# astra-vision/rain-rendering

Hardware: AMD Instinct MI355X
Metric: rainy frames/sec @ 1242x375, 100 mm/hr (higher is better)
Workload: dtype f64 alpha/mask, f32 colour

## Files before the change

rain-rendering_amd/csrc/rainhip.hip:

```cpp
#include <hip/hip_runtime.h>

#include <dlfcn.h>

#include <cstddef>
#include <cstdio>
#include <cstdlib>
#include <algorithm>
#include <cstring>
#include <string>
#include <mutex>
#include <unordered_map>
#include <vector>

#include "rainhip.h"
#include "rr_device.h"
#include "rr_prepass.h"
#include "rr_deflate.h"
#include "rr_pngrows.h"
#include "rr_particles.h"

using namespace rr;

namespace {

// ... 88 lines not shown
    out[1] = __hiloint2double((int)q.d, (int)q.c);
    out[2] = __hiloint2double((int)q.f, (int)q.e);
  } else if (kind == 1) {
    out[0] = (double)__uint_as_float(q.a);
    out[1] = (double)__uint_as_float(q.b);
    out[2] = (double)__uint_as_float(q.c);
  } else {
    out[0] = (double)q.a / 255.0;
    out[1] = (double)q.b / 255.0;
    out[2] = (double)q.c / 255.0;
  }
}
__device__ inline int bg_kind(const FrameDesc& fr) { return (fr.in_types & RR_IN_BG_U8) ? 2 : ((fr.in_types & RR_IN_BG_F32) ? 1 : 0); }
__device__ inline int rainy_kind(const FrameDesc& fr) {
  if (fr.rainy_bg == fr.bg) return bg_kind(fr);
  return (fr.in_types & RR_IN_RAINY_U8) ? 2 : ((fr.in_types & RR_IN_RAINY_F32) ? 1 : 0);
}
typedef float float2_u __attribute__((ext_vector_type(2), aligned(4)));
typedef float float4_u __attribute__((ext_vector_type(4), aligned(4)));

__device__ inline void wave_lds_sync() {
  __builtin_amdgcn_fence(__ATOMIC_ACQ_REL, "wavefront");
  __builtin_amdgcn_wave_barrier();
}

#ifdef RR_PHASES
__device__ unsigned long long g_phase[8][8];
#define PH_DECL unsigned long long ph_t0_ = __builtin_readcyclecounter(), ph_acc_[8] = {0, 0, 0, 0, 0, 0, 0, 0};
#define PH_WAITVM asm volatile("s_waitcnt vmcnt(0)" ::: "memory");
#define PH(k)                                                   \
  {                                                             \
    const unsigned long long ph_n_ = __builtin_readcyclecounter(); \
    ph_acc_[k] += ph_n_ - ph_t0_;                               \
    ph_t0_ = ph_n_;                                             \
  }
#define PH_FLUSH(kid)                                           \
  if ((threadIdx.x & 63) == 0) {                                \
    for (int ph_q_ = 0; ph_q_ < 8; ph_q_++)                     \
      if (ph_acc_[ph_q_]) atomicAdd(&g_phase[kid][ph_q_], ph_acc_[ph_q_]); \
  }
#define PH_PARAMS , unsigned long long& ph_t0_, unsigned long long (&ph_acc_)[8]
#define PH_PASS , ph_t0_, ph_acc_
#define PH_COUNT(k) ph_acc_[k] += 1;
#else
#define PH_PARAMS
#define PH_PASS
#define PH_COUNT(k)
#define PH_DECL
#define PH_WAITVM
#define PH(k)
#define PH_FLUSH(kid)
#endif

struct Scratch {
  DropPlan* plan;
  CompRec* comp;
  CompRec32* comp32;
  int32_t* poly;
  int32_t* npts;
  int64_t* sizes;
  double* prefix;
  double* fband;
  double* arena;
  double* partial;
  double* means;
  int64_t* arena_need;
  int32_t* overflow;
  unsigned long long* need_max;
  int32_t* list_rot;
  int32_t* rot_total;
  int32_t* list_gen;
  int32_t* list_slow;
  int4* blur_items;
  int32_t* list_small;
  double* colpart;
  double* wtab;
  double* wtab_big;
  const uint8_t* tex_pad;
  const int64_t* tex_poff;
  uint4* fov_erec;
  uint32_t* fov_pix;
  int32_t* fov_list;
  int32_t* fov_list_n;
  uint4* fov_rec;
  int32_t* fov_order;
  int32_t* fov_slot;
  int32_t fov_slots;
  uint8_t* blended;
  int32_t* pad_first;
  int32_t* eff_first;
  uint32_t* spans;
  int4* bbox;
  uint16_t* clist;
  int32_t* ccount;
  int32_t* counts;
  int32_t* list_big;
  int32_t* big_off;
  int32_t* bigs_list;
  int32_t* bigs_n;
  uint4* tkey;
  uint4* lrec;
  int32_t* canon;
  int32_t* htab;
  int32_t blur_bx, blur_by;
  int32_t* rows_list;
  int32_t* rows_n;
  int32_t* rows_hist;
  unsigned long long* rows_cost;
  int32_t* rows_next;
  int32_t* rows_bounds;
  int32_t* rows_fbase;
  int32_t* rows_sorted;
  const uint8_t* tex_pair;
  const int64_t* tex_qoff;
  int32_t colpart_f32;
  int32_t rows_on, n_tex;
  int32_t big_on, n_buckets;
};

__global__ __launch_bounds__(256) void k_env_prefix(const FrameDesc* frames, Dims dm, double* prefix) {
  const int lane = threadIdx.x & 63;
  const int row = blockIdx.x * 4 + (threadIdx.x >> 6), f = blockIdx.y;
  if (row >= dm.He) return;
  const FrameDesc& fr = frames[f];
  const int We = dm.We;
  const bool e32 = (fr.in_types & RR_IN_ENV_F32) != 0;
  const global_ptr<const double> env = as_global(static_cast<const double*>(fr.env)) + (int64_t)row * We * 3;
  const global_ptr<const double> om = as_global(static_cast<const double*>(fr.omega)) + (int64_t)row * We;
// ... 885 lines not shown
    int32_t* dst = pass == 0 ? slot : order;
    const int shift = 16 + 8 * pass;
    for (int e = t; e < 256 * FOV_SORT_WAVES; e += 64 * FOV_SORT_WAVES) s_cnt[e] = 0u;
    __syncthreads();
    for (int p = p0 + lane; p < p1; p += 64) {
      const int idx = pass == 0 ? p : src[p];
      atomicAdd(&s_cnt[((recs[idx].w >> shift) & 255u) * FOV_SORT_WAVES + wave], 1u);
    }
    __syncthreads();
    {
      uint32_t c[4], sum = 0u;
#pragma unroll
      for (int k = 0; k < 4; k++) { c[k] = s_cnt[4 * t + k]; sum += c[k]; }
      const uint32_t incl = wave_incl_scan_u32(sum);
      if (lane == 63) s_wtot[wave] = incl;
      __syncthreads();
      uint32_t run = incl - sum;
      for (int w = 0; w < wave; w++) run += s_wtot[w];
#pragma unroll
      for (int k = 0; k < 4; k++) { s_cnt[4 * t + k] = run; run += c[k]; }
    }
    __syncthreads();
    for (int c = p0; c < p1; c += 64) {
      const int p = c + lane;
      const bool valid = p < p1;
      const int idx = valid ? (pass == 0 ? p : src[p]) : 0;
      const uint32_t digit = valid ? (recs[idx].w >> shift) & 255u : 0u;
      unsigned long long peers = __ballot(valid);
#pragma unroll
      for (int b = 0; b < 8; b++) {
        const bool bit = (digit >> b) & 1u;
        const unsigned long long bal = __ballot(bit);
        peers &= bit ? bal : ~bal;
      }
      const int rank = __popcll(peers & ((1ull << lane) - 1ull)), np = __popcll(peers);
      uint32_t* cnt = &s_cnt[digit * FOV_SORT_WAVES + wave];
      const uint32_t at = *cnt;
      wave_lds_sync();
      if (valid) {
        dst[at + rank] = idx;
        if (rank == np - 1) *cnt = at + (uint32_t)np;
      }
      wave_lds_sync();
    }
    __syncthreads();
  }
  for (int p = t; p < n; p += 64 * FOV_SORT_WAVES) slot[order[p]] = p;
}

template <int DPT, int EMAX, bool E32>
__global__ __launch_bounds__(1024) void k_fov_sums32(const FrameDesc* frames, Dims dm, int max_drops, int Hp, int Dp, int rpb, int nchunk, Scratch sc) {
  extern __shared__ __attribute__((aligned(16))) float s_dyn32[];
  const int We = dm.We;
  float4* s_P = reinterpret_cast<float4*>(s_dyn32);
  float* s_wt = reinterpret_cast<float*>(s_P + (We + 1));
  const int f = blockIdx.y, band = blockIdx.x % COL_PARTS, chunk = blockIdx.x / COL_PARTS;
  const int NT = blockDim.x, t = threadIdx.x, lane = t & 63, nw = NT >> 6;
  const int wave = __builtin_amdgcn_readfirstlane(t >> 6);
  const FrameDesc& fr = frames[f];
  const int n = fr.n_drops;
  const int per = (n + nchunk - 1) / nchunk;
  const int d0 = chunk * per, d1 = imin(n, d0 + per);
  if (d0 >= n) return;
  const int y0 = band * rpb, y1 = imin(dm.He, y0 + rpb);
  const int Cw = (((We + nw - 1) / nw) + 1) & ~1;
  const int cw0 = wave * Cw;
  uint32_t sp[DPT];
  auto drop_of = [&](int i) { return sc.fov_slots ? sc.fov_order[(int64_t)f * max_drops + i] : i; };
#pragma unroll
  for (int d = 0; d < DPT; d++) {
    const int i = d0 + d * NT + t;
    sp[d] = 4u * (uint32_t)((i < d1 && sc.npts[(int64_t)f * max_drops + drop_of(i)] > 0) ? i : max_drops);
  }
  if (t == 0) s_P[0] = make_float4(0.f, 0.f, 0.f, 0.f);
  float S[DPT][4];
  uint32_t any = 0;
#pragma unroll
  for (int d = 0; d < DPT; d++) S[d][0] = S[d][1] = S[d][2] = S[d][3] = 0.f;
  double totY = 0.0, totw = 0.0;
  struct RowRegs {
    float4_u a[EMAX];
    float2_u d[EMAX], w[EMAX];
  };
  typedef uint32_t u32x4 __attribute__((ext_vector_type(4)));
  typedef uint32_t u32x2 __attribute__((ext_vector_type(2)));
  auto descriptor = [](const void* p) {
    return __builtin_amdgcn_make_buffer_rsrc(const_cast<void*>(p), (short)0, 0x7fffffff, 0x00020000);
  };
  const __amdgpu_buffer_rsrc_t rs_env = descriptor(fr.env), rs_om = descriptor(fr.omega);
  const __amdgpu_buffer_rsrc_t rs_sp = descriptor(sc.spans + (int64_t)f * Hp * Dp);
  auto load_row = [&](int y, RowRegs& R) {
#pragma unroll
    for (int e = 0; e < EMAX; e++) {
      const int c = cw0 + e * 128 + 2 * lane;
      const int cb = imax(imin(c, We - 2), 0);
      if (E32) {
        const u32x4 a = __builtin_amdgcn_raw_buffer_load_b128(rs_env, cb * 12, y * We * 12, 0);
        const u32x2 d = __builtin_amdgcn_raw_buffer_load_b64(rs_env, cb * 12 + 16, y * We * 12, 0);
        const u32x2 w = __builtin_amdgcn_raw_buffer_load_b64(rs_om, cb * 4, y * We * 4, 0);
        R.a[e] = float4_u{__uint_as_float(a.x), __uint_as_float(a.y), __uint_as_float(a.z), __uint_as_float(a.w)};
        R.d[e] = float2_u{__uint_as_float(d.x), __uint_as_float(d.y)};
        R.w[e] = float2_u{__uint_as_float(w.x), __uint_as_float(w.y)};
      } else {
        auto f64at = [&](const __amdgpu_buffer_rsrc_t& rs, int voff, int soff) {
          const u32x2 v = __builtin_amdgcn_raw_buffer_load_b64(rs, voff, soff, 0);
          return (float)__hiloint2double((int)v.y, (int)v.x);
        };
        const int so = y * We * 24, vo = cb * 24;
        R.a[e] = float4_u{f64at(rs_env, vo, so), f64at(rs_env, vo + 8, so), f64at(rs_env, vo + 16, so), f64at(rs_env, vo + 24, so)};
        R.d[e] = float2_u{f64at(rs_env, vo + 32, so), f64at(rs_env, vo + 40, so)};
        R.w[e] = float2_u{f64at(rs_om, cb * 8, y * We * 8), f64at(rs_om, cb * 8 + 8, y * We * 8)};
      }
    }
  };
  auto row = [&](int y, RowRegs& R, uint32_t (&cur)[DPT], uint32_t (&nxt)[DPT]) {
    float carry[4] = {0.f, 0.f, 0.f, 0.f};
    float ps[EMAX][4], pa[EMAX][4], pb[EMAX][4];
#pragma unroll
    for (int e = 0; e < EMAX; e++) {
      const int cl = e * 128 + 2 * lane, c = cw0 + cl;
      const bool v0 = cl < Cw && c < We, v1 = cl < Cw && c + 1 < We, last = v0 && !v1;
      const float wa = v0 ? (last ? R.w[e].y : R.w[e].x) : 0.f, wb = v1 ? R.w[e].y : 0.f;
      pa[e][0] = (last ? R.a[e].w : R.a[e].x) * wa; pa[e][1] = (last ? R.d[e].x : R.a[e].y) * wa; pa[e][2] = (last ? R.d[e].y : R.a[e].z) * wa; pa[e][3] = wa;
      pb[e][0] = R.a[e].w * wb; pb[e][1] = R.d[e].x * wb; pb[e][2] = R.d[e].y * wb; pb[e][3] = wb;
    }
    load_row(imin(y + 1, y1 - 1), R);
#pragma unroll
    for (int d = 0; d < DPT; d++) nxt[d] = __builtin_amdgcn_raw_buffer_load_b32(rs_sp, (int)sp[d], imin(y + 1, Hp - 1) * Dp * 4, 0);
#pragma unroll
    for (int e = 0; e < EMAX; e++) {
      if (e * 128 < Cw) {
#pragma unroll
        for (int k = 0; k < 4; k++) {
          const float v = wave_incl_scan_f32(pa[e][k] + pb[e][k]) + carry[k];
          ps[e][k] = v;
          carry[k] = readlane_f32(v, 63);
        }
      }
    }
    if (lane == 0) {
#pragma unroll
      for (int k = 0; k < 4; k++) s_wt[wave * 4 + k] = carry[k];
    }
    __syncthreads();
    float basev[4];
#pragma unroll
    for (int k = 0; k < 4; k++) {
      const float wt = row16_incl_scan_f32(lane < nw ? s_wt[lane * 4 + k] : 0.f);
      const float u = readlane_f32(wt, wave > 0 ? wave - 1 : 0);
      basev[k] = wave > 0 ? u : 0.f;
    }
#pragma unroll
    for (int e = 0; e < EMAX; e++) {
      const int cl = e * 128 + 2 * lane, c = cw0 + cl;
      if (cl < Cw && c < We) {
        float o[4];
#pragma unroll
        for (int k = 0; k < 4; k++) o[k] = basev[k] + ps[e][k];
        s_P[c + 1] = make_float4(o[0] - pb[e][0], o[1] - pb[e][1], o[2] - pb[e][2], o[3] - pb[e][3]);
        if (c + 1 < We) s_P[c + 2] = make_float4(o[0], o[1], o[2], o[3]);
        if (c == We - 1 || c + 1 == We - 1) { totY += (double)o[2]; totw += (double)o[3]; }
      }
    }
    __syncthreads();
#pragma unroll
    for (int d = 0; d < DPT; d++) {
      const uint32_t v = cur[d];
      any |= (v != 0u ? 1u : 0u) << d;
      const float4 h = s_P[v >> 16], l = s_P[v & 0xffffu];
      S[d][0] += h.x - l.x;
      S[d][1] += h.y - l.y;
      S[d][2] += h.z - l.z;
      S[d][3] += h.w - l.w;
    }
#pragma unroll
    for (int d = 0; d < DPT; d++) cur[d] = nxt[d];
  };
  RowRegs RA;
  uint32_t qa[DPT], qb[DPT];
  if (y0 < y1) {
    load_row(y0, RA);
#pragma unroll
    for (int d = 0; d < DPT; d++) qa[d] = __builtin_amdgcn_raw_buffer_load_b32(rs_sp, (int)sp[d], y0 * Dp * 4, 0);
  }
  for (int y = y0; y < y1; y++) row(y, RA, qa, qb);
#pragma unroll
  for (int d = 0; d < DPT; d++) {
    const int i = d0 + d * NT + t;
    if (i < d1) {
      float* o = reinterpret_cast<float*>(sc.colpart) + ((int64_t)(f * COL_PARTS + band) * 5) * max_drops + i;
#pragma unroll
      for (int k = 0; k < 4; k++) o[(int64_t)max_drops * k] = S[d][k];
      o[(int64_t)max_drops * 4] = ((any >> d) & 1u) ? 1.0f : 0.0f;
    }
  }
  {
    const int cl = (We - 1 - cw0) & ~1;
    if (chunk == 0 && We - 1 >= cw0 && cl < Cw && ((cl >> 1) & 63) == lane) {
      sc.fband[(f * COL_PARTS + band) * 2 + 0] = totw;
      sc.fband[(f * COL_PARTS + band) * 2 + 1] = totY;
    }
  }
}

__global__ __launch_bounds__(128) void k_fov_poly_general(const FrameDesc* frames, Dims dm, rr_camera cam, int max_drops, Scratch sc) {
  const int f = blockIdx.y, i = blockIdx.x * blockDim.x + threadIdx.x;
  const FrameDesc& fr = frames[f];
  if (i >= fr.n_drops) return;
  const int64_t gi = (int64_t)f * max_drops + i;
  int32_t* px = sc.poly + gi * 2 * POLY_STRIDE;
  const rr_drop d = load_drop(fr.drops + i);
  int npts = fov_polygon(d, cam, dm.He, dm.We, px, px + POLY_STRIDE);
  if (fr.strategy == 1) npts = -1;
  sc.npts[gi] = npts;
}

__global__ __launch_bounds__(256) void k_fov_sums_general(const FrameDesc* frames, Dims dm, int max_drops, Scratch sc, int cv_rule, int n_fov) {
  const int f = blockIdx.y;
  const int wave = threadIdx.x >> 6, lane = threadIdx.x & 63;
  const int i = blockIdx.x * 4 + wave;
  if (i >= frames[f].n_drops) return;
  const int64_t gi = (int64_t)f * max_drops + i;
  const int n = sc.npts[gi];
  double S[4] = {0, 0, 0, 0};
  int any = 0;
  if (n > 0) {
    const int32_t* px = sc.poly + gi * 2 * POLY_STRIDE;
    const int32_t* py = px + POLY_STRIDE;
    int ymin = lane < n ? py[lane] : 0x7fffffff, ymax = lane < n ? py[lane] : -0x7fffffff;
    for (int ofs = 32; ofs > 0; ofs >>= 1) {
      ymin = min(ymin, __shfl_xor(ymin, ofs));
      ymax = max(ymax, __shfl_xor(ymax, ofs));
    }
    const int ya = max(ymin, 0), yb = min(ymax, dm.He - 1);
    const double* P = sc.prefix + (int64_t)f * dm.He * (int64_t)(dm.We + 1) * 4;
    const bool cv = cv_rule && fov_fill_rule_cv_applies(px, py, n, n_fov, dm.He, dm.We);
    for (int y = ya + lane; y <= yb; y += 64) {
      int xl_, xr_;
      if (cv ? fov_rowspan_cv(px, py, n, y, dm.We, xl_, xr_) : fov_rowspan_fast(px, py, n, y, dm.We, xl_, xr_)) {
        any = 1;
        const double* row = P + (int64_t)y * (dm.We + 1) * 4;
        const double* hi = row + (int64_t)(xr_ + 1) * 4;
        const double* lo = row + (int64_t)xl_ * 4;
        for (int k = 0; k < 4; k++) S[k] += hi[k] - lo[k];
      }
    }
    for (int ofs = 32; ofs > 0; ofs >>= 1) {
      for (int k = 0; k < 4; k++) S[k] += __shfl_xor(S[k], ofs);
      any |= __shfl_xor(any, ofs);
    }
  }
  if (lane == 0) {
    for (int b = 0; b < COL_PARTS; b++) {
      double* o = sc.colpart + ((int64_t)(f * COL_PARTS + b) * 5) * max_drops + i;
      for (int k = 0; k < 4; k++) o[(int64_t)max_drops * k] = b == 0 ? S[k] : 0.0;
      o[(int64_t)max_drops * 4] = b == 0 ? (double)any : 0.0;
    }
  }
}

__global__ __launch_bounds__(256) void k_colour(const FrameDesc* frames, Dims dm, int max_drops, double cam_exposure, Scratch sc) {
  const int f = blockIdx.y;
  const int s = blockIdx.x * 256 + threadIdx.x;
  const FrameDesc& fr = frames[f];
  if (s >= fr.n_drops) return;
  const int i = sc.fov_slots ? sc.fov_order[(int64_t)f * max_drops + s] : s;
  const int64_t gi = (int64_t)f * max_drops + i;
  const DropPlan& p = sc.plan[gi];
  CompRec rec;
  rec.x0 = rec.y0 = rec.x1 = rec.y1 = 0;
  rec.ox = rec.oy = rec.pitch = rec.pad = 0;
  rec.off = 0;
  rec.tau_one = rec.g = 0;
  rec.K[0] = rec.K[1] = rec.K[2] = 0;
  rec.zdist = fr.depth ? fabs(as_global((const double*)fr.drops[i].wps)[2]) : 0.0;
  int status = p.status;
  bool blended = false;
  const int n = sc.npts[gi];
  if (n == 0) status = RR_DROP_FOV_FAIL;
  if (n < 0) {
    if (status == RR_DROP_OK && sc.sizes[gi] > 0) {
      blended = true;
      rec.K[0] = rec.K[1] = rec.K[2] = 1.0;
      rec.x0 = p.vis_x0;
      rec.y0 = p.vis_y0;
      rec.x1 = p.vis_x0 + p.vis_w;
      rec.y1 = p.vis_y0 + p.vis_h;
      rec.ox = -p.vis_x0;
      rec.oy = -p.vis_y0;
      rec.pitch = p.tw;
      rec.off = p.a0_off;
      rec.tau_one = p.tau_one;
      rec.g = p.g;
    }
  }
  if (n > 0) {
    double S[4] = {0, 0, 0, 0};
    bool any = false;
    double sumW = 0.0, sumY = 0.0;
    for (int b = 0; b < COL_PARTS; b++) {
      const int64_t at = ((int64_t)(f * COL_PARTS + b) * 5) * max_drops + s;
      if (sc.colpart_f32) {
        const float* part = reinterpret_cast<const float*>(sc.colpart) + at;
        for (int k = 0; k < 4; k++) S[k] += (double)part[(int64_t)max_drops * k];
        any = any || part[(int64_t)max_drops * 4] != 0.0f;
      } else {
        const double* part = sc.colpart + at;
        for (int k = 0; k < 4; k++) S[k] += part[(int64_t)max_drops * k];
        any = any || part[(int64_t)max_drops * 4] != 0.0;
      }
      sumW += sc.fband[(f * COL_PARTS + b) * 2 + 0];
      sumY += sc.fband[(f * COL_PARTS + b) * 2 + 1];
    }
    if (!any) status = RR_DROP_EMPTY_FOV;
    if (status == RR_DROP_OK && sc.sizes[gi] > 0) {
      blended = true;
      colour_from_sums(S, sumW, sumY / sumW, rec.K);
      if (p.r1 > 0) {
        const int fx0 = p.vis_x0 - p.crop_x + (p.shift - p.r2), fy0 = p.vis_y0 - p.crop_y + (p.shift - p.r1);
        rec.x0 = imax(p.vis_x0, fx0);
        rec.y0 = imax(p.vis_y0, fy0);
        rec.x1 = imin(p.vis_x0 + p.vis_w, fx0 + p.ew);
        rec.y1 = imin(p.vis_y0 + p.vis_h, fy0 + p.eh);
        if (rec.x1 <= rec.x0 || rec.y1 <= rec.y0) { rec.x0 = rec.y0 = rec.x1 = rec.y1 = 0; }
        rec.ox = -(fx0 - p.epad);
        rec.oy = -fy0;
        rec.pitch = p.epitch;
        rec.off = p.a1_off;
      } else {
        const int rx0 = p.vis_x0 - p.crop_x + p.shift, ry0 = p.vis_y0 - p.crop_y + p.shift;
        rec.x0 = imax(p.vis_x0, rx0);
        rec.y0 = imax(p.vis_y0, ry0);
        rec.x1 = imin(p.vis_x0 + p.vis_w, rx0 + p.tw);
        rec.y1 = imin(p.vis_y0 + p.vis_h, ry0 + p.th);
        if (rec.x1 <= rec.x0 || rec.y1 <= rec.y0) { rec.x0 = rec.y0 = rec.x1 = rec.y1 = 0; }
        rec.ox = -rx0;
        rec.oy = -ry0;
        rec.pitch = p.tw;
        rec.off = p.a0_off;
      }
      rec.tau_one = p.tau_one;
      rec.g = p.g;
    }
  }
  {
    const double BIG = 1.0e50;
    const bool tame = fabs(rec.tau_one) < BIG && (rec.tau_one == 0.0 || rec.tau_one > 1.0e-200) && fabs(rec.g) < BIG &&
                      fabs(rec.K[0]) < BIG && fabs(rec.K[1]) < BIG && fabs(rec.K[2]) < BIG && p.kind != KIND_EXT;
    rec.pad = tame ? 0 : 1;
  }
  sc.comp[gi] = rec;
  {
    CompRec32 r32;
    r32.xx = (uint32_t)(rec.x0 & 0xffff) | ((uint32_t)(rec.x1 & 0xffff) << 16);
    r32.yy = (uint32_t)(rec.y0 & 0xffff) | ((uint32_t)(rec.y1 & 0xffff) << 16);
    r32.base = rec.off + ((int64_t)rec.oy * rec.pitch + rec.ox);
    r32.pitch_slow = (uint32_t)rec.pitch | ((uint32_t)(rec.pad ? 1 : 0) << 31);
    r32.te = (float)(rec.tau_one / cam_exposure);
    r32.kg[0] = (float)(rec.K[0] * rec.g); r32.kg[1] = (float)(rec.K[1] * rec.g); r32.kg[2] = (float)(rec.K[2] * rec.g);
    r32.zdist = rec.zdist;
    r32.spare0 = 0;
    r32.spare[0] = r32.spare[1] = r32.spare[2] = r32.spare[3] = 0;
    sc.comp32[gi] = r32;
// ... 3334 lines not shown
      ctx->prof_stats.push_back(s);
    }
    ctx->ev_pool.push_back(pe.a);
    ctx->ev_pool.push_back(pe.b);
  }
  ctx->prof_pending.clear();
}

bool fov_fast_path(const rr_ctx* ctx, const Dims& dm) {
  return !ctx->general_fov && dm.He <= HE_MAX && dm.We <= FOV_WE_MAX && (int64_t)dm.We * dm.He < (1 << 22) && ctx->cam.n_fov * 1 <= 64 &&
         ctx->cam.n_fov >= 3;
}

int ensure_scratch(rr_ctx* ctx, int n, int max_drops, const Dims& dm, bool need_comp_out) {
  const bool grow_frames = n > ctx->cap_frames;
  const bool grow_drops = max_drops > ctx->cap_drops;
  const bool dims_change = dm.H != ctx->cap_dims.H || dm.W != ctx->cap_dims.W || dm.He != ctx->cap_dims.He || dm.We != ctx->cap_dims.We;
  const bool general = !fov_fast_path(ctx, dm);
  if (grow_frames || grow_drops || dims_change || (need_comp_out && !ctx->d_comp_out) || general != ctx->scratch_general || ctx->cam.n_fov > ctx->erec_nfov) {
    HIPCHK(hipDeviceSynchronize());
    const int F = grow_frames ? n : ctx->cap_frames;
    const int D = grow_drops ? max_drops : ctx->cap_drops;
    const size_t fd = (size_t)F * (size_t)(D > 0 ? D : 1);
    const int Hp = (dm.He + 3) & ~3;
    int rc;
    if ((rc = dev_alloc(ctx, ctx->sc.plan, fd))) return rc;
    if ((rc = dev_alloc(ctx, ctx->sc.comp, fd))) return rc;
    if ((rc = dev_alloc(ctx, ctx->sc.comp32, fd))) return rc;
    if ((rc = dev_alloc(ctx, ctx->sc.npts, fd))) return rc;
    if ((rc = dev_alloc(ctx, ctx->sc.sizes, fd))) return rc;
    if ((rc = dev_alloc(ctx, ctx->sc.list_rot, fd))) return rc;
    if ((rc = dev_alloc(ctx, ctx->sc.rows_list, fd))) return rc;
    if ((rc = dev_alloc(ctx, ctx->sc.rows_sorted, fd))) return rc;
    if ((rc = dev_alloc(ctx, ctx->sc.rows_n, (size_t)F * 3))) return rc;
    if ((rc = dev_alloc(ctx, ctx->sc.rows_hist, (size_t)RW_TEX_MAX * 3 + 16))) return rc;
    ctx->sc.rows_cost = reinterpret_cast<unsigned long long*>(ctx->sc.rows_hist + RW_TEX_MAX);
    ctx->sc.rows_next = ctx->sc.rows_hist + 3 * RW_TEX_MAX;
    ctx->sc.rot_total = ctx->sc.rows_next + 1;
    if ((rc = dev_alloc(ctx, ctx->sc.rows_bounds, (size_t)RW_SHARE_MAX + 1))) return rc;
    if ((rc = dev_alloc(ctx, ctx->sc.rows_fbase, (size_t)F * RW_TEX_MAX))) return rc;
    if ((rc = dev_alloc(ctx, ctx->sc.fov_list, fd))) return rc;
    if ((rc = dev_alloc(ctx, ctx->sc.fov_erec, general ? 1 : fd * (size_t)(ctx->cam.n_fov > 0 ? ctx->cam.n_fov : RR_MAX_FOV)))) return rc;
    if ((rc = dev_alloc(ctx, ctx->sc.fov_pix, general ? 1 : fd * (size_t)(ctx->cam.n_fov > 0 ? ctx->cam.n_fov : RR_MAX_FOV)))) return rc;
    ctx->erec_nfov = ctx->cam.n_fov;
    if ((rc = dev_alloc(ctx, ctx->sc.fov_rec, general ? 1 : fd))) return rc;
    if ((rc = dev_alloc(ctx, ctx->sc.fov_order, general ? 1 : fd))) return rc;
    if ((rc = dev_alloc(ctx, ctx->sc.fov_slot, general ? 1 : fd))) return rc;
    if ((rc = dev_alloc(ctx, ctx->sc.fov_list_n, (size_t)F))) return rc;
    if ((rc = dev_alloc(ctx, ctx->sc.list_gen, fd))) return rc;
    if ((rc = dev_alloc(ctx, ctx->sc.list_slow, fd))) return rc;
    if ((rc = dev_alloc(ctx, ctx->sc.blur_items, fd * 8))) return rc;
    if ((rc = dev_alloc(ctx, ctx->sc.list_small, fd))) return rc;
    if ((rc = dev_alloc(ctx, ctx->sc.colpart, fd * COL_PARTS * 5))) return rc;
    if ((rc = dev_alloc(ctx, ctx->sc.wtab, fd * 2 * (BR_MAX + 1)))) return rc;
    if ((rc = dev_alloc(ctx, ctx->sc.wtab_big, (size_t)F * SLOW_CAP * 2 * (MAX_R + 1)))) return rc;
    if (general) {
      if ((rc = dev_alloc(ctx, ctx->sc.poly, fd * 2 * POLY_STRIDE))) return rc;
      if ((rc = dev_alloc(ctx, ctx->sc.prefix, (size_t)F * dm.He * (size_t)(dm.We + 1) * 4))) return rc;
      if ((rc = dev_alloc(ctx, ctx->sc.spans, 1))) return rc;
    } else {
      if ((rc = dev_alloc(ctx, ctx->sc.poly, 1))) return rc;
      if ((rc = dev_alloc(ctx, ctx->sc.prefix, 1))) return rc;
      const size_t per_frame = (size_t)(((D > 0 ? D : 1) + 1 + 7) & ~7) * (size_t)Hp;
      if ((rc = dev_alloc(ctx, ctx->sc.spans, (size_t)F * per_frame))) return rc;
      HIPCHK(hipMemset(ctx->sc.spans, 0, sizeof(uint32_t) * (size_t)F * per_frame));
    }
    ctx->scratch_general = general;
    ctx->scratch_hp = Hp;
    if ((rc = dev_alloc(ctx, ctx->sc.bbox, fd))) return rc;
    if ((rc = dev_alloc(ctx, ctx->sc.blended, fd))) return rc;
    {
      const size_t nct = (size_t)((dm.W + CTILE - 1) / CTILE) * ((dm.H + CTILE - 1) / CTILE);
      if ((rc = dev_alloc(ctx, ctx->sc.clist, fd * nct))) return rc;
      if ((rc = dev_alloc(ctx, ctx->sc.ccount, (size_t)F * nct))) return rc;
    }
    if ((rc = dev_alloc(ctx, ctx->sc.counts, (size_t)F * 8))) return rc;
    if ((rc = dev_alloc(ctx, ctx->sc.canon, fd))) return rc;
    if ((rc = dev_alloc(ctx, ctx->sc.bigs_list, fd))) return rc;
    if ((rc = dev_alloc(ctx, ctx->sc.bigs_n, (size_t)F))) return rc;
    if ((rc = dev_alloc(ctx, ctx->sc.tkey, fd * 2))) return rc;
    if ((rc = dev_alloc(ctx, ctx->sc.lrec, fd))) return rc;
    if ((rc = dev_alloc(ctx, ctx->sc.list_big, fd))) return rc;
    if ((rc = dev_alloc(ctx, ctx->sc.big_off, fd + F))) return rc;
    if ((rc = dev_alloc(ctx, ctx->sc.htab, fd * 2))) return rc;
    if ((rc = dev_alloc(ctx, ctx->sc.fband, (size_t)F * COL_PARTS * 2))) return rc;
    const int ntiles = ((dm.W + TILE - 1) / TILE) * ((dm.H + TILE - 1) / TILE);
    if ((rc = dev_alloc(ctx, ctx->sc.partial, (size_t)F * ntiles * 4))) return rc;
    if ((rc = dev_alloc(ctx, ctx->sc.means, (size_t)F * 4))) return rc;
    if ((rc = dev_alloc(ctx, ctx->sc.arena_need, (size_t)F))) return rc;
    if ((rc = dev_alloc(ctx, ctx->d_frames, (size_t)F))) return rc;
    if ((rc = dev_alloc(ctx, ctx->d_comp_out, (size_t)F * dm.H * dm.W * 3))) return rc;
    if (ctx->arena_cap == 0) ctx->arena_cap = (int64_t)(D > 0 ? D : 1) * 1024 + (1 << 20);
    if ((rc = dev_alloc(ctx, ctx->sc.arena, (size_t)F * (size_t)ctx->arena_cap))) return rc;
    ctx->cap_frames = F;
    ctx->cap_drops = D;
    ctx->cap_dims = dm;
  }
  return RR_OK;
}

int grow_arena(rr_ctx* ctx) {
  HIPCHK(hipDeviceSynchronize());
  unsigned long long need = 0;
  HIPCHK(hipMemcpy(&need, ctx->sc.need_max, sizeof(need), hipMemcpyDeviceToHost));
  if ((int64_t)need > ctx->arena_cap) {
    const int64_t cap = ((int64_t)need + (int64_t)need / 4 + (1 << 16) + 15) & ~15LL;
// ... 164 lines not shown
    const dim3 dgrid((max_drops + 64 * DDA_WAVES - 1) / (64 * DDA_WAVES), n);
    if (fov_dda) {
      ProfScope ps(ctx, fs, "k_fov_vertices");
      HIPCHK(hipMemsetAsync(sc.fov_list_n, 0, sizeof(int32_t) * (size_t)n, fs));
      hipLaunchKernelGGL(k_fov_vertices, dgrid, dim3(64 * DDA_WAVES), 0, fs, ctx->d_frames, dm, ctx->cam, D, ctx->fov_order, sc);
    }
    if (fov_dda) {
      ProfScope ps(ctx, fs, "k_fov_sort");
      hipLaunchKernelGGL(k_fov_sort, dim3(n), dim3(64 * FOV_SORT_WAVES), 0, fs, ctx->d_frames, D, sc);
    }
    if (fast) {
      ProfScope ps(ctx, fs, "k_fov_spans");
      const int G = imin(64 / ctx->cam.n_fov, FOV_GROUPS);
      const bool dda = fov_dda;
      const int v32 = fov32 ? 1 : 0;
      const dim3 grid((max_drops + 4 * G - 1) / (4 * G), n);
      if (dda) {
        hipLaunchKernelGGL(k_fov_dda, dgrid, dim3(64 * DDA_WAVES), 0, fs, ctx->d_frames, dm, ctx->cam, D, Hp, Dp, cv_rule ? 1 : 0, sc);
        const dim3 lgrid(imin((int)grid.x, 8), n);
        if (dm.He <= 384)
          hipLaunchKernelGGL((k_fov_spans<6, true>), lgrid, dim3(256), 0, fs, ctx->d_frames, dm, ctx->cam, D, Hp, Dp, 0, cv_rule ? 1 : 0, sc);
        else if (dm.He <= 512)
          hipLaunchKernelGGL((k_fov_spans<8, true>), lgrid, dim3(256), 0, fs, ctx->d_frames, dm, ctx->cam, D, Hp, Dp, 0, cv_rule ? 1 : 0, sc);
        else
          hipLaunchKernelGGL((k_fov_spans<16, true>), lgrid, dim3(256), 0, fs, ctx->d_frames, dm, ctx->cam, D, Hp, Dp, 0, cv_rule ? 1 : 0, sc);
      } else if (dm.He <= 384)
        hipLaunchKernelGGL((k_fov_spans<6, false>), grid, dim3(256), 0, fs, ctx->d_frames, dm, ctx->cam, D, Hp, Dp, v32, cv_rule ? 1 : 0, sc);
      else if (dm.He <= 512)
        hipLaunchKernelGGL((k_fov_spans<8, false>), grid, dim3(256), 0, fs, ctx->d_frames, dm, ctx->cam, D, Hp, Dp, v32, cv_rule ? 1 : 0, sc);
      else
        hipLaunchKernelGGL((k_fov_spans<16, false>), grid, dim3(256), 0, fs, ctx->d_frames, dm, ctx->cam, D, Hp, Dp, v32, cv_rule ? 1 : 0, sc);
    } else {
      ProfScope ps(ctx, fs, "k_fov_poly");
      hipLaunchKernelGGL(k_fov_poly_general, dim3((max_drops + 127) / 128, n), dim3(128), 0, fs, ctx->d_frames, dm, ctx->cam, D, sc);
    }
    sc.colpart_f32 = (fast && fov32) ? 1 : 0;
    if (fast) {
      ProfScope ps(ctx, fs, "k_fov_sums");
      const size_t row_bytes = ((size_t)(dm.We + 1) * 2 + 16 * 2) * sizeof(double);
      auto passes = [&](int nt) { return ((((dm.We + nt / 64 - 1) / (nt / 64)) + 1) / 2 * 2 + 127) / 128; };
      const int NT = 1024;
      const bool e1 = passes(NT) <= 1;
      const int DPT = ctx->fov_dpt ? ctx->fov_dpt : (max_drops <= NT ? 1 : (max_drops <= 2 * NT ? 2 : (max_drops <= 4 * NT ? 4 : 8)));
      const int rpb = ((dm.He + COL_PARTS - 1) / COL_PARTS + 3) & ~3;
      const int nchunk = (max_drops + NT * DPT - 1) / (NT * DPT);
      const dim3 grid(COL_PARTS * 2 * nchunk, n);
      auto launch = [&](auto kern) -> hipError_t {
        hipError_t e = hipFuncSetAttribute(reinterpret_cast<const void*>(kern), hipFuncAttributeMaxDynamicSharedMemorySize, (int)row_bytes);
        if (e != hipSuccess) return e;
        hipLaunchKernelGGL(kern, grid, dim3(NT), row_bytes, fs, ctx->d_frames, dm, D, Hp, Dp, rpb, nchunk, sc);
        return hipSuccess;
      };
      auto launch32 = [&](auto kern) -> hipError_t {
        const size_t bytes = ((size_t)(dm.We + 1) * 4 + 16 * 4) * sizeof(float);
        hipError_t e = hipFuncSetAttribute(reinterpret_cast<const void*>(kern), hipFuncAttributeMaxDynamicSharedMemorySize, (int)bytes);
        if (e != hipSuccess) return e;
        hipLaunchKernelGGL(kern, dim3(COL_PARTS * nchunk, n), dim3(NT), bytes, fs, ctx->d_frames, dm, D, Hp, Dp, rpb, nchunk, sc);
        return hipSuccess;
      };
      bool all32 = true;
      for (int f = 0; f < n; f++) all32 = all32 && (in[f].in_types & RR_IN_ENV_F32);
      for (int f = 0; f < n && !all32; f++)
        if (in[f].in_types & RR_IN_ENV_F32) {
          ctx->err = "RR_IN_ENV_F32 must be set for every frame of a batch or for none";
          return RR_E_ARG;
        }
      hipError_t e = fov32
                         ? (all32 ? (e1 ? (DPT == 1 ? launch32(k_fov_sums32<1, 1, true>) : DPT == 2 ? launch32(k_fov_sums32<2, 1, true>) : DPT == 4 ? launch32(k_fov_sums32<4, 1, true>) : launch32(k_fov_sums32<8, 1, true>))
                                        : (DPT == 1 ? launch32(k_fov_sums32<1, 2, true>) : DPT == 2 ? launch32(k_fov_sums32<2, 2, true>) : DPT == 4 ? launch32(k_fov_sums32<4, 2, true>) : launch32(k_fov_sums32<8, 2, true>)))
                                  : (e1 ? (DPT == 1 ? launch32(k_fov_sums32<1, 1, false>) : DPT == 2 ? launch32(k_fov_sums32<2, 1, false>) : DPT == 4 ? launch32(k_fov_sums32<4, 1, false>) : launch32(k_fov_sums32<8, 1, false>))
                                        : (DPT == 1 ? launch32(k_fov_sums32<1, 2, false>) : DPT == 2 ? launch32(k_fov_sums32<2, 2, false>) : DPT == 4 ? launch32(k_fov_sums32<4, 2, false>) : launch32(k_fov_sums32<8, 2, false>))))
                     : e1 ? (DPT == 1 ? launch(k_fov_sums<1, 1>) : DPT == 2 ? launch(k_fov_sums<2, 1>) : DPT == 4 ? launch(k_fov_sums<4, 1>) : launch(k_fov_sums<8, 1>))
                        : (DPT == 1 ? launch(k_fov_sums<1, 2>) : DPT == 2 ? launch(k_fov_sums<2, 2>) : DPT == 4 ? launch(k_fov_sums<4, 2>) : launch(k_fov_sums<8, 2>));
      if (e != hipSuccess) {
        ctx->err = std::string("k_fov_sums: ") + hipGetErrorString(e);
        return RR_E_HIP;
      }
    } else {
      {
        ProfScope ps(ctx, fs, "k_env_prefix");
        hipLaunchKernelGGL(k_env_prefix, dim3((dm.He + 3) / 4, n), dim3(256), 0, fs, ctx->d_frames, dm, sc.prefix);
        hipLaunchKernelGGL(k_env_consts, dim3(n), dim3(256), 0, fs, dm, sc.prefix, sc.fband);
      }
      {
        ProfScope ps(ctx, fs, "k_fov_sums_general");
        hipLaunchKernelGGL(k_fov_sums_general, dim3((max_drops + 3) / 4, n), dim3(256), 0, fs, ctx->d_frames, dm, D, sc, ctx->fill_rule, ctx->cam.n_fov);
      }
    }
    {
      ProfScope ps(ctx, bs, "k_plan");
      HIPCHK(hipMemsetAsync(sc.bigs_n, 0, sizeof(int32_t) * (size_t)n, bs));
      hipLaunchKernelGGL(k_plan, dim3((max_drops + 127) / 128, n), dim3(128), 0, bs, ctx->d_frames, dm, ctx->cam, ctx->d_tex_h,
                         ctx->d_tex_w, D, fs == bs ? 1 : 0, sc);
      hipLaunchKernelGGL(k_plan_big, dim3((max_drops + 127) / 128, n), dim3(128), 0, bs, ctx->d_frames, ctx->d_tex_h, ctx->d_tex_w, D, sc);
    }
    {
      ProfScope ps(ctx, bs, "k_scan");
      hipLaunchKernelGGL(k_scan, dim3(n), dim3(1024), 0, bs, ctx->d_frames, D, ctx->arena_cap, sc);
    }
    {
      ProfScope ps(ctx, bs, "k_dedup");
      HIPCHK(hipMemsetAsync(sc.htab, 0, sizeof(int32_t) * 2 * (size_t)n * D, bs));
      HIPCHK(hipMemsetAsync(sc.counts, 0, sizeof(int32_t) * 8 * (size_t)n, bs));
      HIPCHK(hipMemsetAsync(sc.rows_hist, 0, sizeof(int32_t) * (RW_TEX_MAX * 3 + 16), bs));
      hipLaunchKernelGGL(k_dedup, dim3((max_drops + 255) / 256, n), dim3(256), 0, bs, ctx->d_frames, D, n, ctx->dedup ? 1 : 0, sc);
    }
    {
      ProfScope ps(ctx, bs, "k_lists");
      hipLaunchKernelGGL(k_lists, dim3(n), dim3(1024), 0, bs, ctx->d_frames, D, ctx->d_tex_h, ctx->d_tex_w, sc);
      if (sc.rows_on) {
        hipLaunchKernelGGL(k_rows_scatter, dim3(n), dim3(1024), 0, bs, D, sc);
        hipLaunchKernelGGL(k_rows_shares, dim3(1), dim3(1024), 0, bs, rows_wgs * ctx->rows_shares, sc);
      }
    }
    {
      ProfScope ps(ctx, s, "k_tile_generic");
      hipLaunchKernelGGL(k_tile_generic, dim3(imin((max_drops + 3) / 4, imax(2, imin(64, 2048 / n))), n), dim3(256), 0, s, ctx->d_frames, D, ctx->d_tex,
                         ctx->d_tex_h, ctx->d_tex_w, ctx->d_tex_off, ctx->d_ctab, sc);
    }
    {
      ProfScope ps(ctx, s, "k_tile_big");
      hipLaunchKernelGGL(k_tile_big, dim3(sc.big_on ? imax(16, imin(1024, 16384 / n)) : 1024, n), dim3(256), 0, s, ctx->d_frames, D, ctx->d_tex, ctx->d_tex_h, ctx->d_tex_w,
                         ctx->d_tex_off, ctx->d_ctab, sc);
    }
    if (sc.rows_on) {
      ProfScope ps(ctx, s, "k_tile_rows");
      hipLaunchKernelGGL(k_tile_rows, dim3(rows_wgs), dim3(64 * RW_WAVES), 0, s, rows_wgs * ctx->rows_shares, ctx->d_tex_h, ctx->d_tex_w, ctx->d_ctab, sc);
    }
    {
      ProfScope ps(ctx, s, "k_tile");
      const int64_t cap = sc.rows_on ? 2048 : 16384;
      hipLaunchKernelGGL(k_tile, dim3((unsigned)std::max<int64_t>(1, std::min<int64_t>((int64_t)n * max_drops, cap))), dim3(256), 0, s, ctx->d_frames, D, ctx->d_tex,
                         ctx->d_tex_h, ctx->d_tex_w, ctx->d_tex_off, sc);
    }
    {
      ProfScope ps(ctx, s, "k_blur_weights");
      hipLaunchKernelGGL(k_blur_weights, dim3((2 * max_drops + 256 / BW_LANES - 1) / (256 / BW_LANES), n), dim3(256), 0, s, ctx->d_frames, D, sc);
    }
    {
      ProfScope ps(ctx, s, "k_blur_small");
// ... 628 lines not shown
  }
  *out = ctx;
  return RR_OK;
}

int rr_destroy(rr_ctx* ctx) {
  if (!ctx) return RR_E_ARG;
  hipSetDevice(ctx->device);
  hipDeviceSynchronize();
  if (ctx->own_tex) hipFree(ctx->d_tex);
  hipFree(ctx->d_tex_h);
  hipFree(ctx->d_tex_w);
  hipFree(ctx->d_tex_off);
  hipFree(ctx->d_tex_pad);
  hipFree(ctx->d_tex_poff);
  hipFree(ctx->d_ctab);
  hipFree(ctx->d_lut);
  hipFree(ctx->sc.plan);
  hipFree(ctx->sc.comp);
  hipFree(ctx->sc.comp32);
  hipFree(ctx->sc.poly);
  hipFree(ctx->sc.npts);
  hipFree(ctx->sc.sizes);
  hipFree(ctx->sc.list_rot);
  hipFree(ctx->sc.fov_erec);
  hipFree(ctx->sc.fov_pix);
  hipFree(ctx->sc.fov_rec);
  hipFree(ctx->sc.fov_order);
  hipFree(ctx->sc.fov_slot);
  hipFree(ctx->sc.rows_list);
  hipFree(ctx->sc.rows_sorted);
  hipFree(ctx->sc.rows_n);
  hipFree(ctx->sc.rows_hist);
  hipFree(ctx->sc.rows_fbase);
  hipFree(ctx->sc.rows_bounds);
  hipFree(ctx->d_tex_pair);
  hipFree(ctx->d_tex_qoff);
  hipFree(ctx->sc.fov_list);
  hipFree(ctx->sc.fov_list_n);
  hipFree(ctx->sc.list_gen);
  hipFree(ctx->sc.list_slow);
  hipFree(ctx->sc.blur_items);
  hipFree(ctx->sc.counts);
  hipFree(ctx->sc.canon);
  hipFree(ctx->sc.bigs_list);
  hipFree(ctx->sc.bigs_n);
  hipFree(ctx->sc.tkey);
  hipFree(ctx->sc.lrec);
  hipFree(ctx->sc.list_big);
  hipFree(ctx->sc.big_off);
  hipFree(ctx->sc.htab);
  hipFree(ctx->sc.list_small);
  hipFree(ctx->sc.colpart);
  hipFree(ctx->sc.wtab);
  hipFree(ctx->sc.wtab_big);
  hipFree(ctx->sc.spans);
  hipFree(ctx->sc.bbox);
  hipFree(ctx->sc.blended);
  hipFree(ctx->d_pad_first);
  hipFree(ctx->d_pngz_slots);
  hipFree(ctx->d_pngz_meta);
  hipFree(ctx->d_eff_first);
  hipFree(ctx->sc.clist);
  hipFree(ctx->sc.ccount);
  hipFree(ctx->sc.prefix);
  hipFree(ctx->sc.fband);
  hipFree(ctx->sc.arena);
  hipFree(ctx->sc.partial);
  hipFree(ctx->sc.means);
  hipFree(ctx->sc.arena_need);
  hipFree(ctx->sc.overflow);
  hipFree(ctx->sc.need_max);
  hipFree(ctx->d_omega);
  hipFree(ctx->d_omega32);
  hipFree(ctx->d_aug);
  hipFree(ctx->d_dgrid);
  hipFree(ctx->d_cdf);
  hipFree(ctx->d_ratio_db);
  hipFree(ctx->d_sims);
  hipFree(ctx->d_traj);
  hipFree(ctx->d_gen_drops);
  hipFree(ctx->d_gen_counts);
  hipFree(ctx->d_field_cnt);
  for (void* b : ctx->noise_blocks) hipFree(b);
  hipFree(ctx->d_noise_desc);
  if (ctx->ev_noise) hipEventDestroy(ctx->ev_noise);
  for (auto* r : {&ctx->ring_frames, &ctx->ring_pre, &ctx->ring_sims, &ctx->ring_noise})
    for (int k = 0; k < rr_ctx::DescRing::N; k++) {
      if (r->host[k]) hipHostFree(r->host[k]);
      if (r->ev[k]) hipEventDestroy(r->ev[k]);
    }
  hipFree(ctx->d_frames);
  hipFree(ctx->d_comp_out);
  for (auto& sl : ctx->slots) {
    hipFree(sl.st.bg);
    hipFree(sl.st.rainy);
    hipFree(sl.st.env);
    hipFree(sl.st.omega);
    hipFree(sl.st.comp);
    hipFree(sl.st.mask);
    hipFree(sl.st.drops);
    hipFree(sl.st.rgb);
    hipFree(sl.st.mask_i);
    hipFree(sl.st.status);
    hipFree(sl.st.colour);
    hipFree(sl.st.ndrops);
// ... 1583 lines not shown
```

Before: 18700.

## Double-buffer fov row prefix sums and split colour part reduction into own kernel

The row loop in k_fov_sums32 now double-buffers the shared prefix array and wave totals. This lets the scan of row y+1 proceed before the lookups of row y, which removes one __syncthreads per row. A new k_fov_reduce kernel sums the per-band column partials once per drop into a ColSum array indexed by drop id. k_colour then reads that array directly instead of looping over the partials through the fov_order indirection. The cost is twice the LDS per block, which can lower occupancy, plus an extra kernel launch and a scratch buffer.

```diff
diff --git a/rain-rendering_amd/csrc/rainhip.hip b/rain-rendering_amd/csrc/rainhip.hip
--- a/rain-rendering_amd/csrc/rainhip.hip
+++ b/rain-rendering_amd/csrc/rainhip.hip
@@ -164,6 +164,11 @@
 #define PH_FLUSH(kid)
 #endif
 
+struct ColSum {
+  double S[4];
+  int32_t any, pad;
+};
+
 struct Scratch {
   DropPlan* plan;
   CompRec* comp;
@@ -186,6 +191,7 @@
   int4* blur_items;
   int32_t* list_small;
   double* colpart;
+  ColSum* colsum;
   double* wtab;
   double* wtab_big;
   const uint8_t* tex_pad;
@@ -1177,8 +1183,8 @@
 __global__ __launch_bounds__(1024) void k_fov_sums32(const FrameDesc* frames, Dims dm, int max_drops, int Hp, int Dp, int rpb, int nchunk, Scratch sc) {
   extern __shared__ __attribute__((aligned(16))) float s_dyn32[];
   const int We = dm.We;
-  float4* s_P = reinterpret_cast<float4*>(s_dyn32);
-  float* s_wt = reinterpret_cast<float*>(s_P + (We + 1));
+  float4* s_P2 = reinterpret_cast<float4*>(s_dyn32);
+  float* s_wt2 = reinterpret_cast<float*>(s_P2 + 2 * (We + 1));
   const int f = blockIdx.y, band = blockIdx.x % COL_PARTS, chunk = blockIdx.x / COL_PARTS;
   const int NT = blockDim.x, t = threadIdx.x, lane = t & 63, nw = NT >> 6;
   const int wave = __builtin_amdgcn_readfirstlane(t >> 6);
@@ -1197,7 +1203,7 @@
     const int i = d0 + d * NT + t;
     sp[d] = 4u * (uint32_t)((i < d1 && sc.npts[(int64_t)f * max_drops + drop_of(i)] > 0) ? i : max_drops);
   }
-  if (t == 0) s_P[0] = make_float4(0.f, 0.f, 0.f, 0.f);
+  if (t == 0) s_P2[0] = s_P2[We + 1] = make_float4(0.f, 0.f, 0.f, 0.f);
   float S[DPT][4];
   uint32_t any = 0;
 #pragma unroll
@@ -1238,9 +1244,10 @@
       }
     }
   };
-  auto row = [&](int y, RowRegs& R, uint32_t (&cur)[DPT], uint32_t (&nxt)[DPT]) {
+  float ps[EMAX][4], pb[EMAX][4];
+  auto scan = [&](int y, RowRegs& R, uint32_t (&q)[DPT]) {
     float carry[4] = {0.f, 0.f, 0.f, 0.f};
-    float ps[EMAX][4], pa[EMAX][4], pb[EMAX][4];
+    float pa[EMAX][4];
 #pragma unroll
     for (int e = 0; e < EMAX; e++) {
       const int cl = e * 128 + 2 * lane, c = cw0 + cl;
@@ -1251,7 +1258,7 @@
     }
     load_row(imin(y + 1, y1 - 1), R);
 #pragma unroll
-    for (int d = 0; d < DPT; d++) nxt[d] = __builtin_amdgcn_raw_buffer_load_b32(rs_sp, (int)sp[d], imin(y + 1, Hp - 1) * Dp * 4, 0);
+    for (int d = 0; d < DPT; d++) q[d] = __builtin_amdgcn_raw_buffer_load_b32(rs_sp, (int)sp[d], y * Dp * 4, 0);
 #pragma unroll
     for (int e = 0; e < EMAX; e++) {
       if (e * 128 < Cw) {
@@ -1264,10 +1271,14 @@
       }
     }
     if (lane == 0) {
+      float* s_wt = s_wt2 + (y & 1) * 64;
 #pragma unroll
       for (int k = 0; k < 4; k++) s_wt[wave * 4 + k] = carry[k];
     }
-    __syncthreads();
+  };
+  auto prefix = [&](int y) {
+    const float* s_wt = s_wt2 + (y & 1) * 64;
+    float4* s_P = s_P2 + (y & 1) * (We + 1);
     float basev[4];
 #pragma unroll
     for (int k = 0; k < 4; k++) {
@@ -1287,7 +1298,9 @@
         if (c == We - 1 || c + 1 == We - 1) { totY += (double)o[2]; totw += (double)o[3]; }
       }
     }
-    __syncthreads();
+  };
+  auto lookups = [&](int y, const uint32_t (&cur)[DPT]) {
+    const float4* s_P = s_P2 + (y & 1) * (We + 1);
 #pragma unroll
     for (int d = 0; d < DPT; d++) {
       const uint32_t v = cur[d];
@@ -1298,17 +1311,25 @@
       S[d][2] += h.z - l.z;
       S[d][3] += h.w - l.w;
     }
-#pragma unroll
-    for (int d = 0; d < DPT; d++) cur[d] = nxt[d];
   };
-  RowRegs RA;
-  uint32_t qa[DPT], qb[DPT];
   if (y0 < y1) {
+    RowRegs RA;
+    uint32_t qa[DPT], qb[DPT];
     load_row(y0, RA);
-#pragma unroll
-    for (int d = 0; d < DPT; d++) qa[d] = __builtin_amdgcn_raw_buffer_load_b32(rs_sp, (int)sp[d], y0 * Dp * 4, 0);
-  }
-  for (int y = y0; y < y1; y++) row(y, RA, qa, qb);
+    scan(y0, RA, qa);
+    __syncthreads();
+    prefix(y0);
+    for (int y = y0; y + 1 < y1; y++) {
+      scan(y + 1, RA, qb);
+      __syncthreads();
+      prefix(y + 1);
+      lookups(y, qa);
+#pragma unroll
+      for (int d = 0; d < DPT; d++) qa[d] = qb[d];
+    }
+    __syncthreads();
+    lookups(y1 - 1, qa);
+  }
 #pragma unroll
   for (int d = 0; d < DPT; d++) {
     const int i = d0 + d * NT + t;
@@ -1384,12 +1405,36 @@
   }
 }
 
+__global__ __launch_bounds__(256) void k_fov_reduce(const FrameDesc* frames, int max_drops, Scratch sc) {
+  const int f = blockIdx.y;
+  const int s = blockIdx.x * 256 + threadIdx.x;
+  if (s >= imin(frames[f].n_drops, max_drops)) return;
+  const int i = sc.fov_slots ? sc.fov_order[(int64_t)f * max_drops + s] : s;
+  ColSum r;
+  r.S[0] = r.S[1] = r.S[2] = r.S[3] = 0.0;
+  r.pad = 0;
+  bool any = false;
+  for (int b = 0; b < COL_PARTS; b++) {
+    const int64_t at = ((int64_t)(f * COL_PARTS + b) * 5) * max_drops + s;
+    if (sc.colpart_f32) {
+      const float* part = reinterpret_cast<const float*>(sc.colpart) + at;
+      for (int k = 0; k < 4; k++) r.S[k] += (double)part[(int64_t)max_drops * k];
+      any = any || part[(int64_t)max_drops * 4] != 0.0f;
+    } else {
+      const double* part = sc.colpart + at;
+      for (int k = 0; k < 4; k++) r.S[k] += part[(int64_t)max_drops * k];
+      any = any || part[(int64_t)max_drops * 4] != 0.0;
+    }
+  }
+  r.any = any ? 1 : 0;
+  sc.colsum[(int64_t)f * max_drops + i] = r;
+}
+
 __global__ __launch_bounds__(256) void k_colour(const FrameDesc* frames, Dims dm, int max_drops, double cam_exposure, Scratch sc) {
   const int f = blockIdx.y;
-  const int s = blockIdx.x * 256 + threadIdx.x;
+  const int i = blockIdx.x * 256 + threadIdx.x;
   const FrameDesc& fr = frames[f];
-  if (s >= fr.n_drops) return;
-  const int i = sc.fov_slots ? sc.fov_order[(int64_t)f * max_drops + s] : s;
+  if (i >= fr.n_drops) return;
   const int64_t gi = (int64_t)f * max_drops + i;
   const DropPlan& p = sc.plan[gi];
   CompRec rec;
@@ -1420,20 +1465,11 @@
     }
   }
   if (n > 0) {
-    double S[4] = {0, 0, 0, 0};
-    bool any = false;
+    const ColSum& cs = sc.colsum[gi];
+    double S[4] = {cs.S[0], cs.S[1], cs.S[2], cs.S[3]};
+    const bool any = cs.any != 0;
     double sumW = 0.0, sumY = 0.0;
     for (int b = 0; b < COL_PARTS; b++) {
-      const int64_t at = ((int64_t)(f * COL_PARTS + b) * 5) * max_drops + s;
-      if (sc.colpart_f32) {
-        const float* part = reinterpret_cast<const float*>(sc.colpart) + at;
-        for (int k = 0; k < 4; k++) S[k] += (double)part[(int64_t)max_drops * k];
-        any = any || part[(int64_t)max_drops * 4] != 0.0f;
-      } else {
-        const double* part = sc.colpart + at;
-        for (int k = 0; k < 4; k++) S[k] += part[(int64_t)max_drops * k];
-        any = any || part[(int64_t)max_drops * 4] != 0.0;
-      }
       sumW += sc.fband[(f * COL_PARTS + b) * 2 + 0];
       sumY += sc.fband[(f * COL_PARTS + b) * 2 + 1];
     }
@@ -4874,6 +4910,7 @@
     if ((rc = dev_alloc(ctx, ctx->sc.blur_items, fd * 8))) return rc;
     if ((rc = dev_alloc(ctx, ctx->sc.list_small, fd))) return rc;
     if ((rc = dev_alloc(ctx, ctx->sc.colpart, fd * COL_PARTS * 5))) return rc;
+    if ((rc = dev_alloc(ctx, ctx->sc.colsum, fd))) return rc;
     if ((rc = dev_alloc(ctx, ctx->sc.wtab, fd * 2 * (BR_MAX + 1)))) return rc;
     if ((rc = dev_alloc(ctx, ctx->sc.wtab_big, (size_t)F * SLOW_CAP * 2 * (MAX_R + 1)))) return rc;
     if (general) {
@@ -5144,7 +5181,7 @@
         return hipSuccess;
       };
       auto launch32 = [&](auto kern) -> hipError_t {
-        const size_t bytes = ((size_t)(dm.We + 1) * 4 + 16 * 4) * sizeof(float);
+        const size_t bytes = 2 * ((size_t)(dm.We + 1) * 4 + 16 * 4) * sizeof(float);
         hipError_t e = hipFuncSetAttribute(reinterpret_cast<const void*>(kern), hipFuncAttributeMaxDynamicSharedMemorySize, (int)bytes);
         if (e != hipSuccess) return e;
         hipLaunchKernelGGL(kern, dim3(COL_PARTS * nchunk, n), dim3(NT), bytes, fs, ctx->d_frames, dm, D, Hp, Dp, rpb, nchunk, sc);
@@ -5178,6 +5215,10 @@
         ProfScope ps(ctx, fs, "k_fov_sums_general");
         hipLaunchKernelGGL(k_fov_sums_general, dim3((max_drops + 3) / 4, n), dim3(256), 0, fs, ctx->d_frames, dm, D, sc, ctx->fill_rule, ctx->cam.n_fov);
       }
+    }
+    {
+      ProfScope ps(ctx, fs, "k_fov_reduce");
+      hipLaunchKernelGGL(k_fov_reduce, dim3((max_drops + 255) / 256, n), dim3(256), 0, fs, ctx->d_frames, D, sc);
     }
     {
       ProfScope ps(ctx, bs, "k_plan");
@@ -5912,6 +5953,7 @@
   hipFree(ctx->sc.htab);
   hipFree(ctx->sc.list_small);
   hipFree(ctx->sc.colpart);
+  hipFree(ctx->sc.colsum);
   hipFree(ctx->sc.wtab);
   hipFree(ctx->sc.wtab_big);
   hipFree(ctx->sc.spans);
```

Result: no change. 18850, median of 6 (+0.8%).
